# thomasneff/AdaNeRF

Measured on NVIDIA H100. Metric: frames_per_sec_800x800, higher is better.
Workload: dtype bf16

## Files before the change

### adanerf_b200/csrc/mlp.cu

```cuda
#include <cuda_bf16.h>
#include <cuda_runtime.h>

#include "mlp.cuh"
#include "posenc.cuh"
#include "ptx.cuh"
#include "tiles.cuh"

namespace adn {

template <uint8_t V>
struct ConstFlags {
  __device__ constexpr operator uint8_t() const { return V; }
};

template <int NSPLIT>
struct MlpCfg {
  static constexpr int kNB = (NSPLIT == 2) ? 4 : 5;
  static constexpr int kStageBytes = NSPLIT * kBlkBytes;
  static constexpr int kStages = (NSPLIT == 2) ? 2 : 8;
  static constexpr size_t kActBytes = size_t(NSPLIT) * kNB * kBlkBytes;
  static constexpr size_t kSmemBytes =
      kActBytes + size_t(kStages) * kStageBytes + size_t(kSideFloats) * 4 + 2 * kStages * 8 + 1024 ;
};
static_assert(MlpCfg<1>::kSmemBytes <= 232448 && MlpCfg<2>::kSmemBytes <= 232448, "shared memory per block (sm_90)");

template <bool VIEW>
__device__ __forceinline__ void encode_row(const EncodeParams& enc, long long i, long long rows, uint8_t* blk, int row) {
  float f[64];
#pragma unroll
  for (int k = 0; k < 64; ++k) f[k] = 0.0f;
  if (i < rows) {
    long long ray;
    float zw;
    if (enc.ray_idx) {
      ray = enc.ray_idx[i];
      zw = enc.z[i];
    } else {
      ray = i / enc.K;
      zw = enc.zlut_dense[i - ray * enc.K];
    }
    float pos[3], dir[3];
    sample_inputs(enc.sc, false, enc.ray_o, enc.ray_d, ray, zw, pos, dir);
    if (VIEW) posenc3<4>(dir, f);
    else posenc3<10>(pos, f);
  }
#pragma unroll
  for (int ch = 0; ch < 8; ++ch) pack_chunk8(f + ch * 8, uint32_t(row), ch, blk, nullptr);
}

__device__ __forceinline__ void copy_rows(const uint8_t* __restrict__ src, uint32_t dst, int nblk, int wg, int tw) {
  for (int b = 0; b < nblk; ++b) {
    const uint4* s = reinterpret_cast<const uint4*>(src + size_t(b) * kBlkBytes + size_t(wg) * (kBlkBytes / 2));
    const uint32_t d = dst + uint32_t(b) * kBlkBytes + uint32_t(wg) * (kBlkBytes / 2);
    uint4 v[4];
#pragma unroll
    for (int j = 0; j < 4; ++j) v[j] = __ldg(s + tw + 128 * j);
#pragma unroll
    for (int j = 0; j < 4; ++j) st_shared_v4(d + uint32_t(tw + 128 * j) * 16u, v[j].x, v[j].y, v[j].z, v[j].w);
  }
}

template <int NSPLIT, bool ENC>
__global__ void __launch_bounds__(kMlpThreads, 1)
mlp_kernel(const __grid_constant__ MlpProgram prog, const uint8_t* __restrict__ wblob, const uint8_t* __restrict__ in_tiles,
           float* __restrict__ out, const long long* __restrict__ rows_dev, long long rows_host, int* err_flag,
           const __grid_constant__ EncodeParams enc) {
  static_assert(!ENC || NSPLIT == 1, "fused input encoder: shading net (plain bf16) only");
  using Cfg = MlpCfg<NSPLIT>;
  constexpr int NB = Cfg::kNB;
  constexpr int STAGES = Cfg::kStages;
  constexpr int STAGE_BYTES = Cfg::kStageBytes;
  constexpr int kConsumerWarps = 8, kProducerWarp = 8;

  extern __shared__ uint8_t smem_raw[];
  uint8_t* smem = smem_raw + ((1024u - (smem_u32(smem_raw) & 1023u)) & 1023u);
  uint8_t* act = smem;
  uint8_t* ring = act + Cfg::kActBytes;
  float* side = reinterpret_cast<float*>(ring + size_t(STAGES) * STAGE_BYTES);
  uint64_t* w_full = reinterpret_cast<uint64_t*>(side + kSideFloats);
  uint64_t* w_empty = w_full + STAGES;

  const int warp = __shfl_sync(0xffffffffu, int(threadIdx.x >> 5), 0);
  const int lane = threadIdx.x & 31;
  const long long rows = rows_dev ? *rows_dev : rows_host;
  const long long n_tiles = (rows + kTileM - 1) / kTileM;

  for (int i = threadIdx.x; i < kSideFloats; i += blockDim.x) side[i] = prog.side[i];
  if (threadIdx.x == 0) {
    for (int s = 0; s < STAGES; ++s) {
      mbar_init(&w_full[s], 1);
      mbar_init(&w_empty[s], kConsumerWarps);
    }
    mbar_fence_init();
  }
  __syncthreads();

  if (warp >= kProducerWarp) {
    setmaxnreg_dec<40>();
    if (warp == kProducerWarp && lane == 0) {
      int stage = 0;
      uint32_t phase = 0;
      for (long long t = blockIdx.x; t < n_tiles; t += gridDim.x) {
        for (int l = 0; l < prog.n_layers; ++l) {
          const MlpLayer& L = prog.layers[l];
          const int n_st = int(L.n_kb) * int(L.n_half);
          for (int i = 0; i < n_st; ++i) {
            mbar_wait(&w_empty[stage], phase ^ 1, err_flag, 1);
            mbar_arrive_expect_tx(&w_full[stage], STAGE_BYTES);
            bulk_g2s(ring + size_t(stage) * STAGE_BYTES, wblob + L.w_off + size_t(i) * STAGE_BYTES, STAGE_BYTES, &w_full[stage]);
            if (++stage == STAGES) {
              stage = 0;
              phase ^= 1;
            }
          }
        }
      }
    }
    return;
  }

  setmaxnreg_inc<232>();
  const int wg = warp >> 2;
  const int tw = threadIdx.x & 127;
  const int r0 = 64 * wg + 16 * (warp & 3) + (lane >> 2);
  const int cq = 2 * (lane & 3);
  const int bar_id = 1 + wg;
  const uint32_t act_s = smem_u32(act);
  const uint32_t ring_s = smem_u32(ring);
  const uint32_t wg_off = uint32_t(wg) * (kBlkBytes / 2);
  auto blk_addr = [&](int term, int blk) -> uint32_t { return act_s + uint32_t(term * NB + blk) * kBlkBytes; };
  const uint64_t desc_hi = make_desc_sw128(0) & ~uint64_t(0x3FFF);
  auto desc = [&](uint32_t addr) -> uint64_t { return desc_hi | uint64_t((addr & 0x3FFFF) >> 4); };

  int stage = 0;
  uint32_t phase = 0;
  for (long long t = blockIdx.x; t < n_tiles; t += gridDim.x) {
    if (ENC) {
      if (tw < 64) encode_row<false>(enc, t * kTileM + 64 * wg + tw, rows, act, 64 * wg + tw);
    } else {
#pragma unroll
      for (int term = 0; term < NSPLIT; ++term)
        copy_rows(in_tiles + size_t(t) * prog.in.tile_bytes() + prog.in.blk_off(term, 0), blk_addr(term, 0), prog.in_nblk0, wg, tw);
    }
    fence_proxy_async_smem();
    named_bar_sync(bar_id, 128);
    float alpha[2] = {0.0f, 0.0f};
    for (int l = 0; l < prog.n_layers; ++l) {
      const MlpLayer& L = prog.layers[l];
      float acc[2][64];
      int prev = -1;
#pragma unroll
      for (int nh = 0; nh < 2; ++nh) {
        if (nh >= L.n_half) break;
        for (int kb = 0; kb < L.n_kb; ++kb) {
          const uint32_t a_hi = blk_addr(0, L.a_blk[kb]) + wg_off;
          const uint32_t a_lo = a_hi + uint32_t(NSPLIT - 1) * NB * kBlkBytes;
          const uint32_t b_hi = ring_s + uint32_t(stage) * STAGE_BYTES;
          const uint32_t b_lo = b_hi + uint32_t(NSPLIT - 1) * kBlkBytes;
          const int nk = L.k_cnt[kb];
          mbar_wait(&w_full[stage], phase, err_flag, 2);
          wgmma_fence();
#pragma unroll
          for (int k = 0; k < 4; ++k) {
            if (k < nk) {
              wgmma_m64n128_bf16(acc[nh], desc(a_hi + 32 * k), desc(b_hi + 32 * k), (kb > 0 || k > 0) ? 1u : 0u);
              if (NSPLIT == 2) {
                wgmma_m64n128_bf16(acc[nh], desc(a_lo + 32 * k), desc(b_hi + 32 * k), 1u);
                wgmma_m64n128_bf16(acc[nh], desc(a_hi + 32 * k), desc(b_lo + 32 * k), 1u);
              }
            }
          }
          wgmma_commit();
          wgmma_wait<1>();
          if (prev >= 0 && lane == 0) mbar_arrive(&w_empty[prev]);
          prev = stage;
          if (++stage == STAGES) {
            stage = 0;
            phase ^= 1;
          }
        }
      }
      wgmma_wait<0>();
      if (lane == 0) mbar_arrive(&w_empty[prev]);
      named_bar_sync(bar_id, 128);

      auto epilogue = [&](auto flags) {
        float rgb[2][3] = {{0.f, 0.f, 0.f}, {0.f, 0.f, 0.f}};
#pragma unroll
        for (int nh = 0; nh < 2; ++nh) {
          if (nh >= L.n_half) break;
#pragma unroll
          for (int i = 0; i < 16; ++i) {
            const int col = nh * 128 + 8 * i + cq;
            const float2 b = *reinterpret_cast<const float2*>(side + L.bias_off + col);
#pragma unroll
            for (int rr = 0; rr < 2; ++rr) {
              const int row = r0 + 8 * rr;
              float v0 = acc[nh][4 * i + 2 * rr] + b.x;
              float v1 = acc[nh][4 * i + 2 * rr + 1] + b.y;
              if (flags & LF_FINAL_RAW) {
                const long long grow = t * kTileM + row;
                if (grow < rows) *reinterpret_cast<float2*>(out + grow * prog.out_cols + col) = make_float2(v0, v1);
                continue;
              }
              if (flags & LF_RELU) {
                v0 = fmaxf(v0, 0.0f);
                v1 = fmaxf(v1, 0.0f);
              }
              if (flags & LF_ALPHA_DOT) {
                const float2 w = *reinterpret_cast<const float2*>(side + prog.alpha_w_off + col);
                alpha[rr] = fmaf(v1, w.y, fmaf(v0, w.x, alpha[rr]));
              }
              if (flags & LF_OUT_ACT) {
                const uint32_t off = uint32_t(L.out_blk0 + (col >> 6)) * kBlkBytes + sw128_offset(uint32_t(row), uint32_t(col & 63));
                const uint32_t hi = bf16x2(v0, v1);
                *reinterpret_cast<uint32_t*>(act + off) = hi;
                if (NSPLIT == 2) *reinterpret_cast<uint32_t*>(act + NB * kBlkBytes + off) = bf16x2_lo(v0, v1, hi);
              }
              if (flags & LF_FINAL_RGB) {
#pragma unroll
                for (int k = 0; k < 3; ++k) {
                  const float2 w = *reinterpret_cast<const float2*>(side + prog.rgb_w_off + k * 128 + col);
                  rgb[rr][k] = fmaf(v1, w.y, fmaf(v0, w.x, rgb[rr][k]));
                }
              }
            }
          }
        }
        if (flags & LF_FINAL_RGB) {
#pragma unroll
          for (int rr = 0; rr < 2; ++rr) {
            float a = alpha[rr], c0 = rgb[rr][0], c1 = rgb[rr][1], c2 = rgb[rr][2];
#pragma unroll
            for (int m = 1; m <= 2; m <<= 1) {
              a += __shfl_xor_sync(0xffffffffu, a, m);
              c0 += __shfl_xor_sync(0xffffffffu, c0, m);
              c1 += __shfl_xor_sync(0xffffffffu, c1, m);
              c2 += __shfl_xor_sync(0xffffffffu, c2, m);
            }
            const long long grow = t * kTileM + r0 + 8 * rr;
            if ((lane & 3) == 0 && grow < rows)
              reinterpret_cast<float4*>(out)[grow] = make_float4(c0 + side[prog.rgb_b_off], c1 + side[prog.rgb_b_off + 1],
                                                                 c2 + side[prog.rgb_b_off + 2], a + side[prog.alpha_b_off]);
          }
        }
      };
      using F = uint8_t;
      constexpr F kEpiFlags = LF_RELU | LF_ALPHA_DOT | LF_OUT_ACT | LF_FINAL_RAW | LF_FINAL_RGB;
      switch (L.flags & kEpiFlags) {
        case LF_RELU | LF_OUT_ACT: epilogue(ConstFlags<LF_RELU | LF_OUT_ACT>{}); break;
        case LF_RELU | LF_OUT_ACT | LF_ALPHA_DOT: epilogue(ConstFlags<LF_RELU | LF_OUT_ACT | LF_ALPHA_DOT>{}); break;
        case LF_OUT_ACT: epilogue(ConstFlags<LF_OUT_ACT>{}); break;
        case LF_RELU | LF_FINAL_RGB: epilogue(ConstFlags<LF_RELU | LF_FINAL_RGB>{}); break;
        case LF_FINAL_RAW: epilogue(ConstFlags<LF_FINAL_RAW>{}); break;
        default: epilogue(F(L.flags)); break;
      }
      if (L.flags & LF_LOAD_IN1_AFTER) {
        if (ENC) {
          if (tw < 64) encode_row<true>(enc, t * kTileM + 64 * wg + tw, rows, act, 64 * wg + tw);
        } else {
          copy_rows(in_tiles + size_t(t) * prog.in.tile_bytes() + prog.in.blk_off(0, prog.in_nblk0), blk_addr(0, 0), 1, wg, tw);
        }
      }
      fence_proxy_async_smem();
      named_bar_sync(bar_id, 128);
    }
  }
}

__global__ void pack_rows_kernel(const float* __restrict__ x, long long rows_host, const long long* __restrict__ rows_dev,
                                 int n_feat, const __grid_constant__ TileFormat fmt, uint8_t* __restrict__ tiles) {
  const long long rows = rows_dev ? *rows_dev : rows_host;
  const long long n_tiles = (rows + kTileM - 1) / kTileM;
  const long long total = n_tiles * kTileM * fmt.n_blk * 8;
  for (long long i = blockIdx.x * (long long)blockDim.x + threadIdx.x; i < total; i += (long long)gridDim.x * blockDim.x) {
    const int chunk = int(i & 7);
    const long long rb = i >> 3;
    const int blk = int(rb % fmt.n_blk);
    const long long row = rb / fmt.n_blk;
    const long long t = row >> 7;
    pack_tile_chunk(fmt, tiles + size_t(t) * fmt.tile_bytes(), blk, uint32_t(row & (kTileM - 1)), chunk,
                    [&](int c) { return row < rows ? x[row * n_feat + c] : 0.0f; });
  }
}

cudaError_t set_max_dyn_smem_once(const void* func, int bytes, unsigned long long* done) {
  int dev = 0;
  cudaError_t e = cudaGetDevice(&dev);
  if (e != cudaSuccess) return e;
  if (dev < 64 && ((__atomic_load_n(done, __ATOMIC_ACQUIRE) >> dev) & 1ull)) return cudaSuccess;
  e = cudaFuncSetAttribute(func, cudaFuncAttributeMaxDynamicSharedMemorySize, bytes);
  if (e != cudaSuccess) return e;
  if (dev < 64) __atomic_fetch_or(done, 1ull << dev, __ATOMIC_RELEASE);
  return cudaSuccess;
}

template <int NSPLIT, bool ENC>
static cudaError_t launch_mlp_t(const MlpProgram& prog, const uint8_t* wblob, const uint8_t* in_tiles, float* out,
                                const long long* rows_dev, long long rows_host, int* err_flag, int num_sms, cudaStream_t stream,
                                const EncodeParams& enc) {
  static unsigned long long attr_done = 0;
  const size_t smem = MlpCfg<NSPLIT>::kSmemBytes;
  auto kernel = mlp_kernel<NSPLIT, ENC>;
  cudaError_t e = set_max_dyn_smem_once(reinterpret_cast<const void*>(kernel), int(smem), &attr_done);
  if (e != cudaSuccess) return e;
  long long grid = num_sms;
  if (!rows_dev) {
    const long long n_tiles = (rows_host + kTileM - 1) / kTileM;
    if (n_tiles < grid) grid = n_tiles < 1 ? 1 : n_tiles;
  }
  kernel<<<unsigned(grid), kMlpThreads, smem, stream>>>(prog, wblob, in_tiles, out, rows_dev, rows_host, err_flag, enc);
  return cudaGetLastError();
}

cudaError_t launch_mlp(const MlpProgram& prog, const uint8_t* wblob, const uint8_t* in_tiles, float* out,
                       const long long* rows_dev, long long rows_host, int* err_flag, int num_sms, cudaStream_t stream,
                       const EncodeParams* enc) {
  if (enc) {
    if (prog.in.n_terms != 1) return cudaErrorInvalidValue;
    return launch_mlp_t<1, true>(prog, wblob, in_tiles, out, rows_dev, rows_host, err_flag, num_sms, stream, *enc);
  }
  if (prog.in.n_terms == 2) return launch_mlp_t<2, false>(prog, wblob, in_tiles, out, rows_dev, rows_host, err_flag, num_sms, stream, EncodeParams{});
  return launch_mlp_t<1, false>(prog, wblob, in_tiles, out, rows_dev, rows_host, err_flag, num_sms, stream, EncodeParams{});
}

cudaError_t launch_pack_rows(const float* x, long long rows, const long long* rows_dev, int n_feat, const TileFormat& fmt,
                             uint8_t* tiles, int num_sms, cudaStream_t stream) {
  long long work = ((rows + kTileM - 1) / kTileM) * kTileM * fmt.n_blk * 8;
  int grid = int((work + 255) / 256);
  if (grid < 1) grid = 1;
  if (grid > 16 * num_sms) grid = 16 * num_sms;
  pack_rows_kernel<<<grid, 256, 0, stream>>>(x, rows, rows_dev, n_feat, fmt, tiles);
  return cudaGetLastError();
}

}
```

### adanerf_b200/csrc/ptx.cuh

```cuda
#pragma once
#include <cstdint>
#include <cuda_runtime.h>

namespace adn {

__device__ __forceinline__ uint32_t smem_u32(const void* p) {
  return static_cast<uint32_t>(__cvta_generic_to_shared(p));
}

__device__ __forceinline__ bool elect_one() {
  uint32_t pred;
  asm volatile("{\n\t.reg .pred p;\n\telect.sync _|p, 0xffffffff;\n\tselp.b32 %0, 1, 0, p;\n\t}" : "=r"(pred));
  return pred != 0;
}

__device__ __forceinline__ void st_shared_v4(uint32_t addr, uint32_t x, uint32_t y, uint32_t z, uint32_t w) {
  asm volatile("st.shared.v4.b32 [%0], {%1, %2, %3, %4};" ::"r"(addr), "r"(x), "r"(y), "r"(z), "r"(w) : "memory");
}

__device__ __forceinline__ float4 ld_shared_f4(uint32_t addr) {
  float4 v;
  asm volatile("ld.shared.v4.f32 {%0, %1, %2, %3}, [%4];" : "=f"(v.x), "=f"(v.y), "=f"(v.z), "=f"(v.w) : "r"(addr));
  return v;
}

__device__ __forceinline__ void named_bar_sync(int id, int nthreads) {
  asm volatile("bar.sync %0, %1;" ::"r"(id), "r"(nthreads) : "memory");
}
__device__ __forceinline__ void named_bar_arrive(int id, int nthreads) {
  asm volatile("bar.arrive %0, %1;" ::"r"(id), "r"(nthreads) : "memory");
}

__device__ __forceinline__ void mbar_init(uint64_t* bar, uint32_t count) {
  asm volatile("mbarrier.init.shared::cta.b64 [%0], %1;" ::"r"(smem_u32(bar)), "r"(count) : "memory");
}
__device__ __forceinline__ void mbar_fence_init() {
  asm volatile("fence.mbarrier_init.release.cluster;" ::: "memory");
}
__device__ __forceinline__ void mbar_arrive(uint64_t* bar) {
  asm volatile("{\n\t.reg .b64 st;\n\tmbarrier.arrive.shared::cta.b64 st, [%0];\n\t}" ::"r"(smem_u32(bar)) : "memory");
}
__device__ __forceinline__ void mbar_arrive_expect_tx(uint64_t* bar, uint32_t bytes) {
  asm volatile("{\n\t.reg .b64 st;\n\tmbarrier.arrive.expect_tx.shared::cta.b64 st, [%0], %1;\n\t}" ::"r"(smem_u32(bar)),
               "r"(bytes)
               : "memory");
}
__device__ __forceinline__ bool mbar_try_wait(uint64_t* bar, uint32_t parity) {
  uint32_t ok;
  asm volatile(
      "{\n\t.reg .pred p;\n\t"
      "mbarrier.try_wait.parity.shared::cta.b64 p, [%1], %2, %3;\n\t"
      "selp.b32 %0, 1, 0, p;\n\t}"
      : "=r"(ok)
      : "r"(smem_u32(bar)), "r"(parity), "r"(0x989680u)
      : "memory");
  return ok != 0;
}

#ifndef ADN_WATCHDOG_CYCLES
#define ADN_WATCHDOG_CYCLES (4000000000ll)
#endif
static __device__ __forceinline__ void mbar_wait_slow(uint64_t* bar, uint32_t parity, int* err_flag, int site) {
  const long long t0 = clock64();
  while (!mbar_try_wait(bar, parity)) {
    if (clock64() - t0 > ADN_WATCHDOG_CYCLES) {
      if (err_flag) atomicExch(err_flag, 0x1000 + site);
      __threadfence_system();
      asm volatile("trap;");
    }
  }
}
__device__ __forceinline__ void mbar_wait(uint64_t* bar, uint32_t parity, int* err_flag, int site) {
  if (mbar_try_wait(bar, parity)) return;
  mbar_wait_slow(bar, parity, err_flag, site);
}

__device__ __forceinline__ void bulk_g2s(void* smem_dst, const void* gmem_src, uint32_t bytes, uint64_t* bar) {
  asm volatile("cp.async.bulk.shared::cluster.global.mbarrier::complete_tx::bytes [%0], [%1], %2, [%3];" ::"r"(
                   smem_u32(smem_dst)),
               "l"(gmem_src), "r"(bytes), "r"(smem_u32(bar))
               : "memory");
}
__device__ __forceinline__ void bulk_s2g(void* gmem_dst, const void* smem_src, uint32_t bytes) {
  asm volatile("cp.async.bulk.global.shared::cta.bulk_group [%0], [%1], %2;" ::"l"(gmem_dst), "r"(smem_u32(smem_src)), "r"(bytes)
               : "memory");
}
__device__ __forceinline__ void bulk_commit() { asm volatile("cp.async.bulk.commit_group;" ::: "memory"); }
__device__ __forceinline__ void bulk_wait_read_all() { asm volatile("cp.async.bulk.wait_group.read 0;" ::: "memory"); }
__device__ __forceinline__ void bulk_wait_all() { asm volatile("cp.async.bulk.wait_group 0;" ::: "memory"); }

__device__ __forceinline__ void fence_proxy_async_all() { asm volatile("fence.proxy.async;" ::: "memory"); }
__device__ __forceinline__ void fence_proxy_async_smem() {
  asm volatile("fence.proxy.async.shared::cta;" ::: "memory");
}

template <int N>
__device__ __forceinline__ void setmaxnreg_inc() { asm volatile("setmaxnreg.inc.sync.aligned.u32 %0;" ::"n"(N)); }
template <int N>
__device__ __forceinline__ void setmaxnreg_dec() { asm volatile("setmaxnreg.dec.sync.aligned.u32 %0;" ::"n"(N)); }

__device__ __forceinline__ void wgmma_fence() { asm volatile("wgmma.fence.sync.aligned;" ::: "memory"); }
__device__ __forceinline__ void wgmma_commit() { asm volatile("wgmma.commit_group.sync.aligned;" ::: "memory"); }
template <int N>
__device__ __forceinline__ void wgmma_wait() { asm volatile("wgmma.wait_group.sync.aligned %0;" ::"n"(N) : "memory"); }

__device__ __forceinline__ void wgmma_m64n128_bf16(float (&d)[64], uint64_t a_desc, uint64_t b_desc, uint32_t accumulate) {
  asm volatile(
      "{\n\t.reg .pred p;\n\tsetp.ne.b32 p, %66, 0;\n\t"
      "wgmma.mma_async.sync.aligned.m64n128k16.f32.bf16.bf16 "
      "{%0, %1, %2, %3, %4, %5, %6, %7, %8, %9, %10, %11, %12, %13, %14, %15, "
      "%16, %17, %18, %19, %20, %21, %22, %23, %24, %25, %26, %27, %28, %29, %30, %31, "
      "%32, %33, %34, %35, %36, %37, %38, %39, %40, %41, %42, %43, %44, %45, %46, %47, "
      "%48, %49, %50, %51, %52, %53, %54, %55, %56, %57, %58, %59, %60, %61, %62, %63}, "
      "%64, %65, p, 1, 1, 0, 0;\n\t}"
      : "+f"(d[0]), "+f"(d[1]), "+f"(d[2]), "+f"(d[3]), "+f"(d[4]), "+f"(d[5]), "+f"(d[6]), "+f"(d[7]), "+f"(d[8]),
        "+f"(d[9]), "+f"(d[10]), "+f"(d[11]), "+f"(d[12]), "+f"(d[13]), "+f"(d[14]), "+f"(d[15]), "+f"(d[16]),
        "+f"(d[17]), "+f"(d[18]), "+f"(d[19]), "+f"(d[20]), "+f"(d[21]), "+f"(d[22]), "+f"(d[23]), "+f"(d[24]),
        "+f"(d[25]), "+f"(d[26]), "+f"(d[27]), "+f"(d[28]), "+f"(d[29]), "+f"(d[30]), "+f"(d[31]), "+f"(d[32]),
        "+f"(d[33]), "+f"(d[34]), "+f"(d[35]), "+f"(d[36]), "+f"(d[37]), "+f"(d[38]), "+f"(d[39]), "+f"(d[40]),
        "+f"(d[41]), "+f"(d[42]), "+f"(d[43]), "+f"(d[44]), "+f"(d[45]), "+f"(d[46]), "+f"(d[47]), "+f"(d[48]),
        "+f"(d[49]), "+f"(d[50]), "+f"(d[51]), "+f"(d[52]), "+f"(d[53]), "+f"(d[54]), "+f"(d[55]), "+f"(d[56]),
        "+f"(d[57]), "+f"(d[58]), "+f"(d[59]), "+f"(d[60]), "+f"(d[61]), "+f"(d[62]), "+f"(d[63])
      : "l"(a_desc), "l"(b_desc), "r"(accumulate)
      : "memory");
}

__device__ __forceinline__ uint64_t make_desc_sw128(uint32_t smem_addr_bytes) {
  uint64_t d = 0;
  d |= static_cast<uint64_t>((smem_addr_bytes & 0x3FFFF) >> 4);
  d |= static_cast<uint64_t>(1) << 16;
  d |= static_cast<uint64_t>(1024 >> 4) << 32;
  d |= static_cast<uint64_t>(1) << 62;
  return d;
}

__host__ __device__ __forceinline__ uint32_t sw128_offset(uint32_t row, uint32_t col) {
  const uint32_t chunk = (col >> 3) ^ (row & 7);
  return (row >> 3) * 1024u + (row & 7) * 128u + chunk * 16u + (col & 7) * 2u;
}

}
```

Before: 62.25.

## Use m64n256 wgmma for full-width layers by pairing adjacent ring stages

Result: faster. 63.66, median of 6 (+2.3%).

```diff
diff --git a/adanerf_b200/csrc/mlp.cu b/adanerf_b200/csrc/mlp.cu
--- a/adanerf_b200/csrc/mlp.cu
+++ b/adanerf_b200/csrc/mlp.cu
@@ -44,8 +44,10 @@
     if (VIEW) posenc3<4>(dir, f);
     else posenc3<10>(pos, f);
   }
-#pragma unroll
-  for (int ch = 0; ch < 8; ++ch) pack_chunk8(f + ch * 8, uint32_t(row), ch, blk, nullptr);
+  uint32_t r = uint32_t(row);
+  asm volatile("" : "+r"(r));
+#pragma unroll
+  for (int ch = 0; ch < 8; ++ch) pack_chunk8(f + ch * 8, r, ch, blk, nullptr);
 }
 
 __device__ __forceinline__ void copy_rows(const uint8_t* __restrict__ src, uint32_t dst, int nblk, int wg, int tw) {
@@ -70,6 +72,8 @@
   constexpr int NB = Cfg::kNB;
   constexpr int STAGES = Cfg::kStages;
   constexpr int STAGE_BYTES = Cfg::kStageBytes;
+  constexpr bool PAIRS = (NSPLIT == 1);
+  static_assert(STAGES % 2 == 0, "a stage pair must not wrap around the ring");
   constexpr int kConsumerWarps = 8, kProducerWarp = 8;
 
   extern __shared__ uint8_t smem_raw[];
@@ -100,18 +104,28 @@
     if (warp == kProducerWarp && lane == 0) {
       int stage = 0;
       uint32_t phase = 0;
+      auto next = [&] {
+        if (++stage == STAGES) {
+          stage = 0;
+          phase ^= 1;
+        }
+      };
       for (long long t = blockIdx.x; t < n_tiles; t += gridDim.x) {
         for (int l = 0; l < prog.n_layers; ++l) {
           const MlpLayer& L = prog.layers[l];
+          const bool pair = PAIRS && L.n_half == 2;
+          if (pair && (stage & 1)) {
+            mbar_wait(&w_empty[stage], phase ^ 1, err_flag, 1);
+            mbar_arrive(&w_full[stage]);
+            next();
+          }
           const int n_st = int(L.n_kb) * int(L.n_half);
           for (int i = 0; i < n_st; ++i) {
+            const int src = pair ? (i & 1) * int(L.n_kb) + (i >> 1) : i;
             mbar_wait(&w_empty[stage], phase ^ 1, err_flag, 1);
             mbar_arrive_expect_tx(&w_full[stage], STAGE_BYTES);
-            bulk_g2s(ring + size_t(stage) * STAGE_BYTES, wblob + L.w_off + size_t(i) * STAGE_BYTES, STAGE_BYTES, &w_full[stage]);
-            if (++stage == STAGES) {
-              stage = 0;
-              phase ^= 1;
-            }
+            bulk_g2s(ring + size_t(stage) * STAGE_BYTES, wblob + L.w_off + size_t(src) * STAGE_BYTES, STAGE_BYTES, &w_full[stage]);
+            next();
           }
         }
       }
@@ -149,9 +163,42 @@
       const MlpLayer& L = prog.layers[l];
       float acc[2][64];
       int prev = -1;
+      const bool pair = PAIRS && L.n_half == 2;
+      if (pair) {
+        if (stage & 1) {
+          mbar_wait(&w_full[stage], phase, err_flag, 2);
+          if (lane == 0) mbar_arrive(&w_empty[stage]);
+          if (++stage == STAGES) {
+            stage = 0;
+            phase ^= 1;
+          }
+        }
+        for (int kb = 0; kb < L.n_kb; ++kb) {
+          const uint32_t a_hi = blk_addr(0, L.a_blk[kb]) + wg_off;
+          const uint32_t b = ring_s + uint32_t(stage) * STAGE_BYTES;
+          const int nk = L.k_cnt[kb];
+          mbar_wait(&w_full[stage], phase, err_flag, 2);
+          mbar_wait(&w_full[stage + 1], phase, err_flag, 2);
+          wgmma_fence();
+#pragma unroll
+          for (int k = 0; k < 4; ++k)
+            if (k < nk) wgmma_m64n256_bf16(acc, desc(a_hi + 32 * k), desc(b + 32 * k), (kb > 0 || k > 0) ? 1u : 0u);
+          wgmma_commit();
+          wgmma_wait<1>();
+          if (prev >= 0 && lane == 0) {
+            mbar_arrive(&w_empty[prev]);
+            mbar_arrive(&w_empty[prev + 1]);
+          }
+          prev = stage;
+          if ((stage += 2) == STAGES) {
+            stage = 0;
+            phase ^= 1;
+          }
+        }
+      }
 #pragma unroll
       for (int nh = 0; nh < 2; ++nh) {
-        if (nh >= L.n_half) break;
+        if (pair || nh >= (PAIRS ? 1 : int(L.n_half))) break;
         for (int kb = 0; kb < L.n_kb; ++kb) {
           const uint32_t a_hi = blk_addr(0, L.a_blk[kb]) + wg_off;
           const uint32_t a_lo = a_hi + uint32_t(NSPLIT - 1) * NB * kBlkBytes;
@@ -181,7 +228,10 @@
         }
       }
       wgmma_wait<0>();
-      if (lane == 0) mbar_arrive(&w_empty[prev]);
+      if (lane == 0) {
+        mbar_arrive(&w_empty[prev]);
+        if (pair) mbar_arrive(&w_empty[prev + 1]);
+      }
       named_bar_sync(bar_id, 128);
 
       auto epilogue = [&](auto flags) {
diff --git a/adanerf_b200/csrc/ptx.cuh b/adanerf_b200/csrc/ptx.cuh
--- a/adanerf_b200/csrc/ptx.cuh
+++ b/adanerf_b200/csrc/ptx.cuh
@@ -125,6 +125,40 @@
       : "memory");
 }
 
+__device__ __forceinline__ void wgmma_m64n256_bf16(float (&d)[2][64], uint64_t a_desc, uint64_t b_desc, uint32_t accumulate) {
+  asm volatile(
+      "{\n\t.reg .pred p;\n\tsetp.ne.b32 p, %130, 0;\n\t"
+      "wgmma.mma_async.sync.aligned.m64n256k16.f32.bf16.bf16 "
+      "{"
+      "%0, %1, %2, %3, %4, %5, %6, %7, %8, %9, %10, %11, %12, %13, %14, %15, "
+      "%16, %17, %18, %19, %20, %21, %22, %23, %24, %25, %26, %27, %28, %29, %30, %31, "
+      "%32, %33, %34, %35, %36, %37, %38, %39, %40, %41, %42, %43, %44, %45, %46, %47, "
+      "%48, %49, %50, %51, %52, %53, %54, %55, %56, %57, %58, %59, %60, %61, %62, %63, "
+      "%64, %65, %66, %67, %68, %69, %70, %71, %72, %73, %74, %75, %76, %77, %78, %79, "
+      "%80, %81, %82, %83, %84, %85, %86, %87, %88, %89, %90, %91, %92, %93, %94, %95, "
+      "%96, %97, %98, %99, %100, %101, %102, %103, %104, %105, %106, %107, %108, %109, %110, %111, "
+      "%112, %113, %114, %115, %116, %117, %118, %119, %120, %121, %122, %123, %124, %125, %126, %127}, "
+      "%128, %129, p, 1, 1, 0, 0;\n\t}"
+      : "+f"(d[0][0]), "+f"(d[0][1]), "+f"(d[0][2]), "+f"(d[0][3]), "+f"(d[0][4]), "+f"(d[0][5]), "+f"(d[0][6]), "+f"(d[0][7]),
+        "+f"(d[0][8]), "+f"(d[0][9]), "+f"(d[0][10]), "+f"(d[0][11]), "+f"(d[0][12]), "+f"(d[0][13]), "+f"(d[0][14]), "+f"(d[0][15]),
+        "+f"(d[0][16]), "+f"(d[0][17]), "+f"(d[0][18]), "+f"(d[0][19]), "+f"(d[0][20]), "+f"(d[0][21]), "+f"(d[0][22]), "+f"(d[0][23]),
+        "+f"(d[0][24]), "+f"(d[0][25]), "+f"(d[0][26]), "+f"(d[0][27]), "+f"(d[0][28]), "+f"(d[0][29]), "+f"(d[0][30]), "+f"(d[0][31]),
+        "+f"(d[0][32]), "+f"(d[0][33]), "+f"(d[0][34]), "+f"(d[0][35]), "+f"(d[0][36]), "+f"(d[0][37]), "+f"(d[0][38]), "+f"(d[0][39]),
+        "+f"(d[0][40]), "+f"(d[0][41]), "+f"(d[0][42]), "+f"(d[0][43]), "+f"(d[0][44]), "+f"(d[0][45]), "+f"(d[0][46]), "+f"(d[0][47]),
+        "+f"(d[0][48]), "+f"(d[0][49]), "+f"(d[0][50]), "+f"(d[0][51]), "+f"(d[0][52]), "+f"(d[0][53]), "+f"(d[0][54]), "+f"(d[0][55]),
+        "+f"(d[0][56]), "+f"(d[0][57]), "+f"(d[0][58]), "+f"(d[0][59]), "+f"(d[0][60]), "+f"(d[0][61]), "+f"(d[0][62]), "+f"(d[0][63]),
+        "+f"(d[1][0]), "+f"(d[1][1]), "+f"(d[1][2]), "+f"(d[1][3]), "+f"(d[1][4]), "+f"(d[1][5]), "+f"(d[1][6]), "+f"(d[1][7]),
+        "+f"(d[1][8]), "+f"(d[1][9]), "+f"(d[1][10]), "+f"(d[1][11]), "+f"(d[1][12]), "+f"(d[1][13]), "+f"(d[1][14]), "+f"(d[1][15]),
+        "+f"(d[1][16]), "+f"(d[1][17]), "+f"(d[1][18]), "+f"(d[1][19]), "+f"(d[1][20]), "+f"(d[1][21]), "+f"(d[1][22]), "+f"(d[1][23]),
+        "+f"(d[1][24]), "+f"(d[1][25]), "+f"(d[1][26]), "+f"(d[1][27]), "+f"(d[1][28]), "+f"(d[1][29]), "+f"(d[1][30]), "+f"(d[1][31]),
+        "+f"(d[1][32]), "+f"(d[1][33]), "+f"(d[1][34]), "+f"(d[1][35]), "+f"(d[1][36]), "+f"(d[1][37]), "+f"(d[1][38]), "+f"(d[1][39]),
+        "+f"(d[1][40]), "+f"(d[1][41]), "+f"(d[1][42]), "+f"(d[1][43]), "+f"(d[1][44]), "+f"(d[1][45]), "+f"(d[1][46]), "+f"(d[1][47]),
+        "+f"(d[1][48]), "+f"(d[1][49]), "+f"(d[1][50]), "+f"(d[1][51]), "+f"(d[1][52]), "+f"(d[1][53]), "+f"(d[1][54]), "+f"(d[1][55]),
+        "+f"(d[1][56]), "+f"(d[1][57]), "+f"(d[1][58]), "+f"(d[1][59]), "+f"(d[1][60]), "+f"(d[1][61]), "+f"(d[1][62]), "+f"(d[1][63])
+      : "l"(a_desc), "l"(b_desc), "r"(accumulate)
+      : "memory");
+}
+
 __device__ __forceinline__ uint64_t make_desc_sw128(uint32_t smem_addr_bytes) {
   uint64_t d = 0;
   d |= static_cast<uint64_t>((smem_addr_bytes & 0x3FFFF) >> 4);
```
